# yilane/rag-project-icd10

Hardware: AMD Instinct MI355X
Metric: queries_per_sec (higher is better)
Workload: dtype f16; 1 GPU; BASELINE configs[1]: 10000 random fp32 768-d queries x 37000x768 corpus, top_k=10, search only (pre-embedded, HBM-resident inputs), level reweight fused; nq_per_gpu=10000, corpus_rows=37000, dim=768, top_k=10, mode=auto, parallelism=single GPU, collective_ranks=1

## Files before the change

### rag_project_icd10_amd/csrc/coarse_flat_kernel.hpp

```cpp
#pragma once
#include "coarse_common.hpp"
#include "flat_partition.hpp"

namespace icd {

struct CoarseFlatArgs {
    const _Float16 *q16;
    const _Float16 *c16;
    int nq;
    int n;
    int n_pad;
    int ctiles;
    int total_units;
    int units_per_wg;
    int pos_period;
    int list_tiles;
    int boot_tiles;
    int sparse_from;
    int P;
    float *part_scores;
    int *part_rows;
    float *bounds;
    unsigned int *shared_thr;
    const int *nq_ptr;
    const int *qlist;
    int nwg_virtual;
    int skip_below;
    unsigned long long *dbg;
    unsigned int *pace;
    int pace_period;
    int pace_epochs;
    int pace_shift;
    int pace_lead;
};

constexpr int CO_BOOT_MIN_TILES = 6;
constexpr int CO_KP_WIDE = 24;
constexpr int CO_BOOT_TILES = 8;
constexpr int PACE_SPIN_LIMIT = 20000;
constexpr int CO_SPARSE_FROM = 40;

template <int KP>
__device__ __forceinline__ float flush_emit_parallel(const char *smem, uint32_t qb, int h, int rot, int nlo, int nhi, float thr,
                                                      bool store, float *out_scores, int *out_rows) {
    constexpr int CAP = 64, HALF = 32;
    float v[HALF];
    uint32_t rw[HALF];
    const int lo_end = nlo, hi_begin = CAP - nhi;
#pragma unroll
    for (int j = 0; j < HALF; ++j) {
        const int slot = HALF * h + ((j + rot) & (HALF - 1));
        const bool valid = slot < lo_end || slot >= hi_begin;
        const float sv = *reinterpret_cast<const float *>(smem + qb + slot * 4);
        rw[j] = *reinterpret_cast<const uint32_t *>(smem + qb + CAP * 4 + slot * 4);
        v[j] = valid ? sv : -INFINITY;
    }
    auto pair_sum = [&](int x) {
        const auto sw = __builtin_amdgcn_permlane32_swap((unsigned)x, (unsigned)x, false, false);
        return x + (int)(h ? sw[0] : sw[1]);
    };
    const int total = nlo + nhi;
    float mx = -INFINITY;
#pragma unroll
    for (int j = 0; j < HALF; ++j) mx = fmaxf(mx, v[j]);
    {
        const auto sw = __builtin_amdgcn_permlane32_swap(__float_as_uint(mx), __float_as_uint(mx), false, false);
// ... 124 lines not shown
        quota_ties = h ? max(0, min(tied, room - min(tied_low_lane, room))) : min(tied, room);
        cut = tie;
    }
    int mine_n = 0;
#pragma unroll
    for (int j = 0; j < HALF; ++j) mine_n += (v[j] > cut) ? 1 : 0;
    mine_n += quota_ties;
    const auto swn = __builtin_amdgcn_permlane32_swap((unsigned)mine_n, (unsigned)mine_n, false, false);
    const int other_n = (int)(h ? swn[0] : swn[1]);
    if (total > KP) {
        int dest = h ? other_n : 0;
        int ties_left = quota_ties;
#pragma unroll
        for (int j = 0; j < HALF; ++j) {
            bool take = v[j] > cut;
            if (!take && ties_left > 0 && v[j] == tie && cnt_lo > KP) { take = true; --ties_left; }
            if (take) {
                *reinterpret_cast<float *>(smem + qb + dest * 4) = v[j];
                *reinterpret_cast<uint32_t *>(smem + qb + CAP * 4 + dest * 4) = rw[j];
                ++dest;
            }
        }
        const int kept = mine_n + other_n;
        st.thr = cut;
        st.kept = kept;
        st.aw0 = h ? qb + (CAP - 1) * 4 : qb + (uint32_t)kept * 4;
        st.aw = st.aw0;
    }
}

constexpr int CF_PRODUCT_VAR = 1 + 2 + 8 + 128 + 16 + 2048 + 32768;
constexpr int CF_CACHED_VAR = CF_PRODUCT_VAR + 2097152 + 4194304;
constexpr int CF_PACED_VAR = CF_PRODUCT_VAR + 67108864;
__host__ __device__ constexpr int cf_ring_stages(int var) { return (var & 1048576) ? 6 : CO_S; }
__host__ __device__ constexpr int cf_lds_bytes(int var) { return cf_ring_stages(var) * CO_STAGE_BYTES + CO_BM * CO_CAP * 8 + ((var & 1048576) ? 0 : 4 * 256); }
#define ICD_CF_STAMP(t) do { __builtin_amdgcn_sched_barrier(0); \
    asm volatile("s_memtime %0\n\ts_waitcnt lgkmcnt(0)" : "=s"(t) :: "memory"); \
    __builtin_amdgcn_sched_barrier(0); } while (0)

template <int D, int VAR = CF_PRODUCT_VAR, int KP = CO_KP, bool PERSIST = false>
__global__ __launch_bounds__(256, 1) void coarse_flat_kernel(CoarseFlatArgs a) {
    constexpr int CO_QUOTA = (CO_CAP - KP) / 2 - CO_CHECK_EVERY;
    static_assert(CO_QUOTA >= 8 && KP + 2 * (CO_QUOTA + CO_CHECK_EVERY) <= CO_CAP, "candidate buffer layout");
    constexpr bool EARLY_THR = (VAR & 1) != 0;
    constexpr bool DMA_SPREAD = (VAR & 2) != 0;
    constexpr bool Q_AGPR = (VAR & 8) != 0;
    constexpr bool PF2 = (VAR & 128) != 0;
    constexpr bool REV_WAIT = (VAR & 4) != 0;
    constexpr bool QUAD = (VAR & 16) != 0;
    constexpr bool SETPRIO = (VAR & 131072) != 0;
    constexpr int EXCH = (VAR & 524288) ? 4 : ((VAR & 262144) ? 2 : 1);
    constexpr bool X16 = (VAR & 32768) != 0;
    static_assert(!X16 || (QUAD && (VAR & 8) != 0 && D % 32 == 0), "the 16x16x32 form is built on the quad select and pinned queries");
    constexpr int EPOCH = ((VAR & 32) && (VAR & 2048)) ? 32 : ((VAR & 32) ? 16 : ((VAR & 2048) ? 24 : 0));
    constexpr bool NOBAR = (VAR & 256) != 0, NOVM = (VAR & 512) != 0, STAMPS = (VAR & 1024) != 0;
    constexpr bool NOPASS = (VAR & 4096) != 0, NOSEL = (VAR & 8192) != 0, NODMA = (VAR & 16384) != 0;
    constexpr bool PAIRBAR = (VAR & 1048576) != 0;
    constexpr bool DMA_WIDE = (VAR & 2097152) != 0;
    constexpr bool BOOT_MED3 = (VAR & 4194304) != 0;
    constexpr bool DIRTY_GUARD = (VAR & 8388608) != 0;
    constexpr bool SPARSE_PRE = (VAR & 16777216) != 0;
    static_assert(!SPARSE_PRE || (QUAD && X16), "the group pre-filter is built on the quad select of the 16x16x32 form");
    static_assert(!DMA_WIDE || (X16 && DMA_SPREAD && PF2 && !NODMA), "the wide spread is built on the product's 16x16x32 stage");
    constexpr bool CLOCKS = (VAR & 33554432) != 0;
    constexpr bool PACE = (VAR & 67108864) != 0;
    static_assert(!PACE || (EARLY_THR && EXCH == 1 && !PERSIST), "the pace poll rides on the early threshold load of every tile");
    static_assert(!(CLOCKS && STAMPS), "one use of the debug buffer at a time");
    constexpr int S = cf_ring_stages(VAR);
    constexpr int VM_MID = NOVM ? 63 : (PAIRBAR ? 4 : 4 * (S - 3));
    constexpr int PRO = PAIRBAR ? 4 : S - 1;
    constexpr int VM_TILE_END = NOVM ? 0 : (PAIRBAR ? (DMA_WIDE ? 6 : 8) : (DMA_WIDE ? 4 * (S - 2) - 2 : 4 * (S - 2)));
    constexpr int KS = D / CO_BK;
    constexpr int NF = D / 16;
    static_assert(KS % S == 0, "ring slot must be a compile-time function of the stage");
    using Ops = Sel2Ops<KP>;
    extern __shared__ __attribute__((aligned(16))) char smem[];

    const int tid = threadIdx.x, lane = tid & 63;
    const int wave = __builtin_amdgcn_readfirstlane(tid >> 6);
    const int c = lane & 31, h = lane >> 5;
    const int q16 = lane & 15, g16 = lane >> 4;
    const int nq_act = PERSIST && a.nq_ptr ? min(__builtin_amdgcn_readfirstlane(*a.nq_ptr), a.nq) : a.nq;
    const int total_units = PERSIST ? ((nq_act + CO_BM - 1) / CO_BM) * a.ctiles : a.total_units;
    const int nwg_logical = PERSIST ? (total_units + a.units_per_wg - 1) / a.units_per_wg : (int)gridDim.x;
    if (PERSIST && nq_act <= a.skip_below) return;
    unsigned long long clk_c0 = 0, clk_r0 = 0;
    if constexpr (CLOCKS) {
        clk_c0 = __builtin_amdgcn_s_memtime();
        clk_r0 = __builtin_amdgcn_s_memrealtime();
        __builtin_amdgcn_s_waitcnt(0xC07F);
    }

    uint32_t src_off[4];
#pragma unroll
    for (int i = 0; i < 4; ++i) {
        const int row_local = (wave * 4 + i) * 8 + (lane >> 3);
        const int piece = (lane & 7) ^ ((row_local >> 1) & 7);
        src_off[i] = (uint32_t)row_local * (uint32_t)(D * 2) + (uint32_t)piece * 16u - (uint32_t)(i * 1024);
    }
    uint32_t rd_off[4];
    if constexpr (X16) {
#pragma unroll
        for (int k2 = 0; k2 < 2; ++k2) rd_off[k2] = (uint32_t)q16 * 128u + (uint32_t)(((4 * k2 + g16) ^ ((q16 >> 1) & 7)) * 16);
        rd_off[2] = rd_off[3] = 0u;
    } else {
        const int sw = (c >> 1) & 7;
#pragma unroll
        for (int s = 0; s < 4; ++s) rd_off[s] = (uint32_t)c * 128u + (uint32_t)(((2 * s + h) ^ sw) * 16);
    }
    auto read_frags = [&](half8 (&f)[4], int ring_slot, int s) {
        if constexpr (X16) {
            const char *sb = smem + ring_slot * CO_STAGE_BYTES + (s & 1) * 8192 + rd_off[s >> 1];
#pragma unroll
            for (int t = 0; t < 4; ++t) f[t] = *reinterpret_cast<const half8 *>(sb + t * 2048);
        } else {
            const char *sb = smem + ring_slot * CO_STAGE_BYTES + rd_off[s];
#pragma unroll
            for (int t = 0; t < 4; ++t) f[t] = *reinterpret_cast<const half8 *>(sb + t * 4096);
        }
    };
    constexpr uint32_t RING_BYTES = (uint32_t)S * CO_STAGE_BYTES;
    const uint32_t wave_qbase = RING_BYTES + (uint32_t)(wave * 32) * Ops::QBYTES;
    const uint32_t wave_scratch = RING_BYTES + (uint32_t)CO_BM * Ops::QBYTES + (uint32_t)wave * 256u;
    unsigned long long st_vm = 0, st_bar = 0, st_body = 0, st_sel = 0, st_tiles = 0, st_prev = 0;
    unsigned long long st_comp[2] = {0, 0}, st_thr = 0, st_boot = 0;
    const int last_tile = a.ctiles - 1;

    half8 qf[NF];
    int cur_mtile = -1;
    for (int vblock = (int)blockIdx.x; vblock < (PERSIST ? nwg_logical : (int)blockIdx.x + 1); vblock += PERSIST ? (int)gridDim.x : 1) {
    const int wg = flat_workgroup_of_block(vblock, nwg_logical, a.pos_period);
    const int u_begin = wg * a.units_per_wg;
    const int u_end = min(total_units, u_begin + a.units_per_wg);
    if (u_begin >= u_end) continue;
    int u = u_begin;
    [[maybe_unused]] bool pacing = false;
    [[maybe_unused]] int pace_cls = 0, pace_members = 0, pace_last_epochs = 0;
    [[maybe_unused]] bool pace_last_mine = false;
    if constexpr (PACE) {
        if (a.pace && a.pace_period > 0) {
            pacing = true;
            pace_cls = wg % a.pace_period;
            pace_members = (nwg_logical - pace_cls + a.pace_period - 1) / a.pace_period;
            const int last_units = total_units - (nwg_logical - 1) * a.units_per_wg;
            pace_last_mine = ((nwg_logical - 1) % a.pace_period) == pace_cls;
            pace_last_epochs = last_units >> a.pace_shift;
        }
    }
    while (u < u_end) {
        const int mtile = u / a.ctiles;
        const int t0 = u - mtile * a.ctiles;
        const int run0 = max(u_begin - mtile * a.ctiles, 0);
        const int run1 = min(u_end - mtile * a.ctiles, a.ctiles);
        const int j = (t0 - run0) / a.list_tiles;
        const int t1 = min(run1, run0 + (j + 1) * a.list_tiles);
        const int ntiles = t1 - t0;
        const int ord = flat_first_ordinal(mtile, wg, a.ctiles, a.units_per_wg, a.list_tiles) + j;
        const int slot0 = mtile * CO_BM;

        if (mtile != cur_mtile) {
            if constexpr (X16) {
#pragma unroll
                for (int gr = 0; gr < 2; ++gr) {
                    int qr = slot0 + wave * 32 + 16 * gr + q16;
                    if (PERSIST && a.qlist) qr = a.qlist[min(qr, nq_act - 1)];
                    const _Float16 *qrow = a.q16 + (size_t)qr * D + 8 * g16;
#pragma unroll
                    for (int s = 0; s < NF / 2; ++s) qf[gr * (NF / 2) + s] = *reinterpret_cast<const half8 *>(qrow + 32 * s);
                }
            } else {
                int qr = slot0 + wave * 32 + c;
                if (PERSIST && a.qlist) qr = a.qlist[min(qr, nq_act - 1)];
                const _Float16 *qrow = a.q16 + (size_t)qr * D + 8 * h;
#pragma unroll
                for (int s = 0; s < NF; ++s) qf[s] = *reinterpret_cast<const half8 *>(qrow + 16 * s);
            }
            if constexpr (Q_AGPR) {
#pragma unroll
                for (int s = 0; s < NF; ++s) asm volatile("" : "+a"(qf[s]));
            }
            cur_mtile = mtile;
        }
        const __amdgpu_buffer_rsrc_t crsrc = __builtin_amdgcn_make_buffer_rsrc(
            const_cast<_Float16 *>(a.c16) + (size_t)t0 * CO_BN * D, 0,
            (int)min((size_t)(a.ctiles - t0) * CO_BN * (size_t)(D * 2), (size_t)0x7FFFFFFF), 0x00020000);
        auto issue_pieces = [&](int g_tile, int g_ks, int ring_slot, auto LO, auto HI) {
            const int trow = min(g_tile, last_tile - t0);
            char *dst = smem + ring_slot * CO_STAGE_BYTES + wave * 4096;
            const uint32_t soff = (uint32_t)trow * (uint32_t)(CO_BN * D * 2) + (uint32_t)g_ks * (CO_BK * 2);
            __attribute__((address_space(3))) void *ldst = (__attribute__((address_space(3))) void *)dst;
            constexpr int lo = decltype(LO)::value, hi = decltype(HI)::value;
            if constexpr (lo <= 0 && 0 < hi) __builtin_amdgcn_raw_ptr_buffer_load_lds(crsrc, ldst, 16, src_off[0], soff, 0, 0);
            if constexpr (lo <= 1 && 1 < hi) __builtin_amdgcn_raw_ptr_buffer_load_lds(crsrc, ldst, 16, src_off[1], soff, 1024, 0);
            if constexpr (lo <= 2 && 2 < hi) __builtin_amdgcn_raw_ptr_buffer_load_lds(crsrc, ldst, 16, src_off[2], soff, 2048, 0);
// ... 433 lines not shown
```

### rag_project_icd10_amd/csrc/finalize.hpp

```cpp
#pragma once
#include "exact_kernel.hpp"
#include "topk_select.hpp"

namespace icd {

constexpr int FIN_MAX_CAND = 512;
constexpr int FIN_MAX_CAND_X = 2048;
constexpr int FIN_MAX_K = 128;
constexpr int FIN_MAX_T = 256;
constexpr int FIN_EF = FIN_MAX_CAND / 64;
constexpr int FIN_EF_X = FIN_MAX_CAND_X / 64;
#ifndef ICD_FIN_WALK
#define ICD_FIN_WALK 8
#endif
constexpr int FIN_WALK = ICD_FIN_WALK;
#ifndef ICD_FIN_OCC
#define ICD_FIN_OCC 7
#endif

struct FinArgs {
    const float *part_scores;
    const int *part_rows;
    const float *bounds;
    long long perm_mul;
    int perm_mod;
    double perm_inv;
    int P, KP;
    int P_dense;
    int sparse_max;
    int dense_one_per_cu;
    int dense_grid, dense_bmq, dense_max_p, n_rows;
    int lds_cand;
    int lists_by_query;
    int skip_below;
    int narrow_check;
    int skip_walk;
    int wide_window;
    int nq;
    const int *nq_ptr;
    const int *qlist;
    int k;
    const float *queries;
    const float *corpus;
    int dim;
    const float *qnorm;
    const int *qexp;
    const unsigned char *qbad;
    float rmax, eps_rel;
    float rmax_unc, eps_f32;
    int cexp;
    int *nflag;
    int *flagged;
    float *thr0;
    int *counters;
    int track_run;
    int *host_counters;
    const int *levels;
    long long id_base;
    const long long *row_map;
    float *out_scores;
    long long *out_ids;
    double *out_adj;
    float *out_adj_raw;
    long long *out_adj_ids;
    int *out_adj_levels;
    const int *groups;
    int *out_levels;
    int *out_groups;
    int *out_adj_groups;
};

__device__ __forceinline__ double level_weight(int level) {
    return level == 1 ? 1.2 : (level == 3 ? 0.8 : 1.0);
}

__device__ __forceinline__ float wave_max_f32(float v) {
    const int ninf = (int)0xff800000u;
#define ICD_DPP_MAX(ctrl, rmask) v = fmaxf(v, __int_as_float(__builtin_amdgcn_update_dpp(ninf, __float_as_int(v), ctrl, rmask, 0xf, false)))
    ICD_DPP_MAX(0x111, 0xf);
    ICD_DPP_MAX(0x112, 0xf);
    ICD_DPP_MAX(0x114, 0xf);
    ICD_DPP_MAX(0x118, 0xf);
    ICD_DPP_MAX(0x142, 0xa);
    ICD_DPP_MAX(0x143, 0xc);
#undef ICD_DPP_MAX
// ... 268 lines not shown
        }
        return;
    }
    const int slot = blockIdx.x * 4 + wave;
    if (slot >= nq) return;
    const int qidx = a.qlist ? a.qlist[slot] : slot;
    if (qidx < 0) return;

    int P = a.P;
    if (a.nq_ptr && a.P_dense > 0 && nq > a.sparse_max)
        P = a.dense_max_p > 0 ? exact_adaptive_chunks(nq, a.dense_bmq, a.dense_grid, a.dense_max_p, a.n_rows, a.dense_one_per_cu) : a.P_dense;
    const int ncand = P * a.KP;
    const int lds_cand = a.lds_cand > 0 ? a.lds_cand : ncand;
    char *wbase = smem + (size_t)wave * fin_wave_lds_bytes(RESCORE, a.dim, lds_cand, EWM);
    u64 *keys = reinterpret_cast<u64 *>(wbase);
    u64 *sorted = keys + fin_key_slots(lds_cand);
    double *adjbuf = reinterpret_cast<double *>(sorted + fin_sorted_slots(EWM));
    float *qvec = reinterpret_cast<float *>(adjbuf + fin_adj_slots(EWM));
    float qn_early = 0.0f;
    int qexp_early = 0;
    unsigned char qbad_early = 0;
    if (RESCORE) {
        qn_early = a.qnorm[qidx];
        qexp_early = a.qexp[qidx];
        qbad_early = a.qbad[qidx];
        const float *qsrc0 = a.queries + (size_t)qidx * a.dim;
        for (int d = lane * 4; d < a.dim; d += 256)
            *reinterpret_cast<float4 *>(qvec + d) = *reinterpret_cast<const float4 *>(qsrc0 + d);
    }

    const int k = a.k;
    const size_t lslot = a.lists_by_query ? (size_t)qidx : (size_t)slot;
    const size_t pbase = lslot * ncand;

    const int T = !RESCORE ? k
                  : (a.wide_window && EWM >= 4) ? (ncand >= 256 ? 256 : (ncand >= 128 ? 128 : 64))
                  : ((EWM >= 4 && k > 64 && ncand >= 256) ? 256 : (EWM >= 2 && k > 32 && ncand >= 128) ? 128 : ((ncand > 128 && k <= 12) ? 32 : 64));
    float tau = -INFINITY;
    if (RESCORE) {
        if (lane < P) {
            const float bd = a.bounds[lslot * P + lane];
            if (bd > -INFINITY) tau = bd + fabsf(bd) * COARSE_KEY_SLACK;
        }
    }
    int nres = 0;
    bool merged = false;
    if constexpr (RESCORE && EWM >= 4) {
        if (T > 64) {
            const float two_eps = 2.0f * fin_eps(a, qn_early, qexp_early);
            nres = ncand <= 128 ? fin_merge_window<2>(a, pbase, ncand, T, k, two_eps, keys, sorted, lane, tau)
                                : fin_merge_window<FIN_EF>(a, pbase, ncand, T, k, two_eps, keys, sorted, lane, tau);
            merged = true;
        }
    }
    if (!merged) {
        int nvalid;
        if (ncand <= 128) nvalid = fin_merge<RESCORE, 2>(a, pbase, ncand, T, keys, sorted, lane, tau);
        else if (!RESCORE && EWM >= 4 && ncand > FIN_MAX_CAND) {
            if constexpr (!RESCORE && EWM >= 4) nvalid = fin_merge<false, FIN_EF_X>(a, pbase, ncand, T, keys, sorted, lane, tau);
            else nvalid = 0;
        }
        else nvalid = fin_merge<RESCORE, FIN_EF>(a, pbase, ncand, T, keys, sorted, lane, tau);
        nres = min(nvalid, T);
    }

    if (RESCORE) {
// ... 300 lines not shown
```

### rag_project_icd10_amd/csrc/icd_search.hip

```cpp
#include <hip/hip_runtime.h>

#include <algorithm>
#include <atomic>
#include <chrono>
#include <cmath>
#include <cstdarg>
#include <cstdio>
#include <cstring>
#include <mutex>
#include <new>
#include <string>
#include <vector>

#include "../../include/icd_search.h"
#include "coarse_flat_kernel.hpp"
#include "attention_kernel.hpp"
#include "exact_kernel.hpp"
#include "finalize.hpp"
#include "group_topk.hpp"
#include "hier_kernel.hpp"
#include "stats_kernel.hpp"
#include "stream_kernel.hpp"
#include "term_lookup.hpp"
#include "search_policy.hpp"
// ... 93 lines not shown
    int device = 0;
    bool opt_permute = true;
    bool opt_probe = true;
    bool opt_center = true;
    int opt_pace_shift = 3, opt_pace_lead = 2;
    bool opt_exact_narrow = true;
    int opt_host_one = 3;
    bool opt_stream_one = true;
    bool opt_family_order = true;
    int opt_wide_from = 48;
    int64_t n = 0, id_base = 0;
    long long *row_map = nullptr;
    int n_pad = 0;
    int dim = 0;
    int max_nq = 0, max_nq_pad = 0, max_k = 0;
    bool fast = false;
    float rmax = 0.f;
    float rmax_scaled = 0.f;
    int cexp = 0;
    float *cmean = nullptr;
    float rmax_unc_scaled = 0.f;
    float mean_share = 0.f;
    int num_cu = 256;
    float *corpus = nullptr;
    _Float16 *c16 = nullptr;
    int *levels = nullptr;
    float *qdev = nullptr;
    _Float16 *q16 = nullptr;
    float *qnorm = nullptr;
    int *qexp = nullptr;
    unsigned char *qbad = nullptr;
    float *thr0 = nullptr;
    unsigned int *shared_thr = nullptr;
    long long perm_mul = 0; int perm_mod = 0;
    float *partc_s = nullptr; int *partc_r = nullptr; float *partc_b = nullptr; size_t partc_cap = 0;
    float *part2_s = nullptr; int *part2_r = nullptr; float *part2_b = nullptr; size_t part2_cap = 0;
    float *partx_s = nullptr; int *partx_r = nullptr; size_t partx_cap = 0;
    float *lists_s = nullptr; int *lists_r = nullptr; size_t lists_cap = 0;
    int *nflag = nullptr; int *flagged = nullptr;
    int fallback_word = 0;
    int *h_nflag = nullptr;
    int *h_nflag_dev = nullptr;
    hipEvent_t ev_nflag = nullptr;
    unsigned int *scratch_u32 = nullptr;
    int *order = nullptr, *order_key = nullptr; unsigned int *order_hist = nullptr;
    float *o_scores = nullptr; long long *o_ids = nullptr;
    double *o_adj = nullptr; float *o_adj_raw = nullptr; long long *o_adj_ids = nullptr; int *o_adj_lv = nullptr;
    char *h_pin = nullptr, *h_pin_dev = nullptr;
    const float *host_q = nullptr;
    bool host_one_call = false;
    unsigned long long done_seq = 0;
    bool done_armed = false;
    size_t bytes_ws = 0;
    int chunks_override = 0;
    SearchPolicy pol;
    std::mutex mu;
    int probe_flagged = -1, probe_left = -1;
    bool pass2_enabled = true;
    bool adapt_enabled = true;
    bool profiling = false;
    int prof_every = 1;
    long prof_tick = 0;
    bool prof_now = false;
    bool capturing = false;
    hipEvent_t evring[EV_RING][NUM_EV + 1] = {};
    bool evring_valid[EV_RING][NUM_EV + 1] = {};
// ... 545 lines not shown
    x->fallback_word = 0;
    rec(x, 3, s);
    ExactArgs a{};
    a.corpus = x->corpus; a.queries = c.dq; a.nq = nq; a.n = (int)x->n; a.dim = x->dim; a.P = pn; a.strided = 1;
    a.rows_per_chunk = 128;
    a.part_scores = x->partx_s; a.part_rows = x->partx_r;
    int rc = launch_exact<32, 1, 4, 62, 16, 2, 16>(x, a, mtx_n, s);
    if (rc) return rc;
    rec(x, 4, s);
    FinArgs g = c.f;
    g.part_scores = x->partx_s; g.part_rows = x->partx_r; g.P = pn; g.KP = 32; g.nq = nq; g.lds_cand = pn * 32;
    g.narrow_check = 1; g.nflag = x->nflag; g.flagged = x->flagged;
    rc = launch_finalize<false>(x, g, s);
    if (rc) return rc;
    rec(x, 5, s);
    return run_exact(c, x->flagged, x->nflag, std::min(c.p_sparse, c.row_tiles), true, c.stream_ok, true, false, nullptr);
}

int search_exact(const SearchCtx &c) {
    icd_index *x = c.x;
    HIP_TRY(hipMemsetAsync(x->nflag, 0, sizeof(int), c.s));
    int px = pick_chunks(c.mtx, c.row_tiles, c.pmax_x, x->num_cu * c.wg_per_cu_x);
    const int rc = fit_chunks(c, &px);
    if (rc) return rc;
    x->last_chunks = px;
    rec(x, 3, c.s);
    return run_exact(c, nullptr, nullptr, px, true, false);
}

struct AutoPlan {
    bool wide_lists;
    bool wide_now;
    bool sparse_off;
    int kp_c;
    int ctiles, U, nwg;
    int pc;
    CoarseFlatArgs a;
    int p2, nwg2;
    CoarseFlatArgs a2;
};

int auto_prep(const SearchCtx &c, int nq_pad) {
    icd_index *x = c.x;
    ConvertArgs cv{};
    cv.src = c.dq; cv.dst = x->q16; cv.rows = c.nq; cv.rows_pad = nq_pad; cv.dim = x->dim; cv.mode = 0;
    cv.norm = x->qnorm; cv.scale_exp = x->qexp; cv.bad = x->qbad; cv.zero_u32 = x->shared_thr; cv.zero_i32 = x->nflag;
    cv.zero_u32b = x->shared_thr + x->max_nq_pad;
    hipLaunchKernelGGL(convert_rows_kernel, dim3((nq_pad + 3) / 4), dim3(256), 0, c.s, cv);
    HIP_TRY(hipGetLastError());
    rec(x, 1, c.s);
    return ICD_OK;
}

int split_class_period(int U, int ctiles, int nwg, int xcd_mode = -1) {
    int period = flat_class_period(U, ctiles);
    const int members = nwg / std::max(1, period);
    int split = (members + 11) / 12;
    if (xcd_mode == 0) period = 0;
    else if (xcd_mode == 1) period = 1 << 30;
    else if (xcd_mode == 2) split = 1;
    if (period > 0 && period < (1 << 20)) period *= std::max(1, split);
    return period;
}

int auto_plan(const SearchCtx &c, int nq_pad, AutoPlan &pl) {
    icd_index *x = c.x;
// ... 9 lines not shown
    const SearchDecision dec = policy_decide(x->pol, x->adapt_enabled, nq, k, x->chunks_override);
    pl.sparse_off = dec.sparse_off;
    pl.wide_now = dec.wide_now;
    pl.kp_c = pl.wide_lists ? CO_KP_WIDE : CO_KP;

    CoarseFlatArgs &a = pl.a;
    a = CoarseFlatArgs{};
    a.q16 = x->q16; a.c16 = x->c16; a.nq = nq; a.n = (int)x->n; a.n_pad = ctiles * 128; a.ctiles = ctiles;
    a.total_units = mtc * ctiles;
    a.boot_tiles = c.ov.flat_boot >= 0 ? c.ov.flat_boot : std::max(1, std::min(CO_BOOT_TILES, 96 / std::max(1, k)));
    a.sparse_from = c.ov.flat_sparse >= 0 ? c.ov.flat_sparse : CO_SPARSE_FROM;
    CoarsePlanIn pin{};
    pin.mtc = mtc; pin.ctiles = ctiles; pin.U = std::max(plan.U, c.ov.flat_u); pin.nq = nq; pin.k = k;
    pin.kp = pl.kp_c; pin.kp2 = CO_KP; pin.max_cand = FIN_MAX_CAND;
    pin.wide_lists = pl.wide_lists; pin.wide_now = pl.wide_now; pin.chunks_override = x->chunks_override;
    pin.pass2 = x->pass2_enabled && x->pol.pass2_armed() && x->part2_s;
    pin.partc_cap = (long long)x->partc_cap; pin.part2_cap = (long long)x->part2_cap;
    pin.max_list_tiles = flat_max_list_tiles(x->dim);
    if (c.ov.flat_list > 0) pin.list_override = c.ov.flat_list;
    const CoarsePlan cp = plan_coarse_lists(pin);
    if (!cp.ok)
        return fail(ICD_ERR_UNSUPPORTED, "coarse pass: no list plan for n=%lld dim=%d nq=%d k=%d (lists per query %d, at most %d tiles per list)",
                    (long long)x->n, x->dim, nq, k, cp.P, pin.max_list_tiles);
    const int U = cp.U;
    pl.U = U; pl.pc = cp.P;
    x->last_chunks = cp.P;
    pl.nwg = (a.total_units + U - 1) / U;
    a.list_tiles = cp.list_tiles;
    a.units_per_wg = U; a.P = cp.P;
    a.pos_period = split_class_period(U, ctiles, pl.nwg, c.ov.xcd_mode);
    a.part_scores = x->partc_s; a.part_rows = x->partc_r; a.bounds = x->partc_b; a.shared_thr = x->shared_thr;
    a.dbg = x->dbg;
    a.nwg_virtual = pl.nwg;
    pl.p2 = 0; pl.nwg2 = 0;
    pl.a2 = CoarseFlatArgs{};
    if (cp.P2 > 0) {
        const int U2 = cp.U2;
        CoarseFlatArgs &a2 = pl.a2;
        pl.p2 = cp.P2;
        a2 = a;
        a2.nq_ptr = nullptr; a2.qlist = nullptr;
        a2.units_per_wg = U2; a2.list_tiles = cp.list_tiles2; a2.P = pl.p2;
        a2.boot_tiles = a.boot_tiles;
        pl.nwg2 = (int)(((long long)mtc * ctiles + U2 - 1) / U2);
        a2.pos_period = split_class_period(U2, ctiles, pl.nwg2);
        a2.nwg_virtual = pl.nwg2;
        a2.part_scores = x->part2_s; a2.part_rows = x->part2_r; a2.bounds = x->part2_b;
        a2.shared_thr = x->shared_thr + x->max_nq_pad;
    }
    return ICD_OK;
}

int auto_coarse(const SearchCtx &c, AutoPlan &pl) {
    icd_index *x = c.x;
    hipStream_t s = c.s;
    CoarseFlatArgs &a = pl.a;
    const int nwg = pl.nwg;
    int rc;
    if (launch_coarse_variant(x, c.ov, a, nwg, s, &rc)) return rc;
    if (x->dim == 1024) return launch_coarse_flat<1024, (CF_PRODUCT_VAR & (3 | 16 | 2048))>(x, a, nwg, s);
    if (pl.wide_lists) return launch_coarse_flat<768, CF_PRODUCT_VAR, CO_KP_WIDE>(x, a, nwg, s);
    if ((size_t)x->n_pad * x->dim * 2 <= COARSE_CACHED_IMAGE_BYTES) return launch_coarse_flat<768, CF_CACHED_VAR>(x, a, nwg, s);
    const int t0 = flat_class_period(pl.U, pl.ctiles);
    const int members0 = t0 > 0 ? nwg / t0 : 0;
    const int epochs = x->opt_pace_shift >= 0 ? (pl.U >> x->opt_pace_shift) + 1 : 0;
    if (x->opt_pace_shift >= 0 && members0 >= 4 && (size_t)t0 * epochs <= PACE_WORDS) {
        a.pace = x->pace; a.pace_period = t0; a.pace_epochs = epochs; a.pace_shift = x->opt_pace_shift; a.pace_lead = std::max(1, x->opt_pace_lead);
        HIP_TRY(hipMemsetAsync(x->pace, 0, (size_t)t0 * epochs * sizeof(unsigned int), s));
    }
    return launch_coarse_flat<768, CF_PACED_VAR>(x, a, nwg, s);
}

int auto_first_finalize(const SearchCtx &c, const AutoPlan &pl, FinArgs &g, bool *wide_fin) {
    icd_index *x = c.x;
    const int nq = c.nq, k = c.k;
    hipStream_t s = c.s;
    g = c.f;
    g.part_scores = x->partc_s; g.part_rows = x->partc_r; g.bounds = x->partc_b; g.P = pl.pc; g.KP = pl.kp_c; g.nq = nq;
    g.perm_mul = x->perm_mul; g.perm_mod = x->perm_mod;
    g.perm_inv = (x->perm_mod > 0 && (double)x->perm_mod * (double)x->perm_mod < 9007199254740992.0) ? 1.0 / (double)x->perm_mod : 0.0;
    *wide_fin = pl.wide_now && k <= 32 && pl.pc * g.KP >= 128;
    if (*wide_fin) g.wide_window = 1;
    if (c.ov.fin_skip_walk) g.skip_walk = 1;
    if (*wide_fin && x->opt_family_order && nq >= 1024) {
        OrderArgs o{};
        o.part_scores = g.part_scores; o.part_rows = g.part_rows; o.P = g.P; o.KP = g.KP; o.nq = nq;
        o.perm_mul = g.perm_mul; o.perm_mod = g.perm_mod; o.perm_inv = g.perm_inv;
        o.shift = 6;
        while (((long long)x->n >> o.shift) >= ORDER_BUCKETS) ++o.shift;
        o.key = x->order_key; o.hist = x->order_hist; o.order = x->order;
        HIP_TRY(hipMemsetAsync(x->order_hist, 0, 2 * ORDER_BUCKETS * sizeof(unsigned int), s));
        hipLaunchKernelGGL(order_keys_kernel, dim3((nq + 3) / 4), dim3(256), 0, s, o);
        hipLaunchKernelGGL(order_scatter_kernel, dim3((nq + 1023) / 1024), dim3(1024), 0, s, o);
        HIP_TRY(hipGetLastError());
        g.qlist = x->order; g.lists_by_query = 1; g.nq = 4 * ((nq + 3) / 4);
    }
    const int rc = *wide_fin ? launch_finalize_t<true, false, 4>(x, g, s) : launch_finalize<true>(x, g, s);
    g.qlist = nullptr; g.lists_by_query = 0; g.nq = nq;
    return rc;
}

int auto_wide_retry(const SearchCtx &c, const FinArgs &g) {
    icd_index *x = c.x;
    FinArgs g2 = g;
    g2.qlist = x->flagged; g2.nq_ptr = x->nflag; g2.lists_by_query = 1; g2.wide_window = 1;
    g2.nflag = x->nflag + 1; g2.flagged = x->flagged + x->max_nq_pad;
    const int rc = launch_finalize_t<true, false, 4>(x, g2, c.s);
    if (rc) return rc;
    x->fallback_word = 1;
    return ICD_OK;
}

int auto_second_pass(const SearchCtx &c, AutoPlan &pl, const FinArgs &g) {
    icd_index *x = c.x;
    hipStream_t s = c.s;
    CoarseFlatArgs &a2 = pl.a2;
    const int w_in = x->fallback_word;
    a2.nq_ptr = x->nflag + w_in;
    a2.qlist = x->flagged + (size_t)w_in * x->max_nq_pad;
    a2.skip_below = PASS2_SKIP;
    const int grid2 = std::max(8, std::min(pl.nwg2, x->num_cu) & ~7);
    int rc;
    if (x->dim == 1024) rc = launch_coarse_flat<1024, (CF_PRODUCT_VAR & (3 | 16 | 2048)), CO_KP, true>(x, a2, grid2, s);
    else rc = launch_coarse_flat<768, CF_PRODUCT_VAR, CO_KP, true>(x, a2, grid2, s);
    if (rc) return rc;
    FinArgs g3 = g;
    g3.part_scores = x->part2_s; g3.part_rows = x->part2_r; g3.bounds = x->part2_b; g3.P = pl.p2; g3.KP = CO_KP;
    g3.qlist = a2.qlist; g3.nq_ptr = a2.nq_ptr; g3.lists_by_query = 0; g3.wide_window = 1; g3.skip_below = PASS2_SKIP;
    g3.nflag = x->nflag + 2; g3.flagged = x->flagged + (size_t)2 * x->max_nq_pad;
    rc = launch_finalize_t<true, false, 4>(x, g3, s);
    if (rc) return rc;
    x->fallback_word = 2;
    x->last_p2 = pl.p2; x->last_p2_word = w_in;
    return ICD_OK;
}

int auto_fallback(const SearchCtx &c, bool sparse_off) {
    icd_index *x = c.x;
    const int *fl_list = x->flagged + (size_t)x->fallback_word * x->max_nq_pad;
    const int *fl_count = x->nflag + x->fallback_word;
    int px = std::min(c.p_sparse, c.row_tiles);
    if (px < c.p_sparse) {
        const int rc = fit_chunks(c, &px);
        if (rc) return rc;
        return run_exact(c, fl_list, fl_count, px, true, false, true, true, c.f.thr0);
    }
    return run_exact(c, fl_list, fl_count, c.p_sparse, true, c.stream_ok, !sparse_off, true, c.f.thr0);
}

int search_auto(const SearchCtx &c) {
    icd_index *x = c.x;
    const int nq_pad = ((c.nq + 127) / 128) * 128;
    int rc = auto_prep(c, nq_pad);
    if (rc) return rc;
    AutoPlan pl;
    rc = auto_plan(c, nq_pad, pl);
    if (rc) return rc;
    rc = auto_coarse(c, pl);
    if (rc) return rc;
    rec(x, 2, c.s);
    FinArgs g;
    bool wide_fin = false;
    rc = auto_first_finalize(c, pl, g, &wide_fin);
    if (rc) return rc;
    x->fallback_word = 0;
    if (!wide_fin && c.k <= 32 && pl.pc * g.KP >= 128) {
        rc = auto_wide_retry(c, g);
        if (rc) return rc;
    }
    if (pl.p2 > 0) {
        rc = auto_second_pass(c, pl, g);
        if (rc) return rc;
    }
    policy_note_search(x->pol, x->adapt_enabled, x->pass2_enabled, c.nq, pl.p2, pl.wide_now, x->chunks_override, pl.pc * pl.kp_c);
    rec(x, 3, c.s);
    return auto_fallback(c, pl.sparse_off);
}

int search_device(icd_index *x, const float *dq, int nq, int k, int mode, const Outs &o, hipStream_t s, const BandArgs *band = nullptr, RowMasks mask = nullptr) {
    const bool use_fast = !band && (mode == ICD_MODE_AUTO) && x->fast && k <= FAST_MAX_K && (x->dim == 768 || x->dim == 1024);
    x->prof_now = !x->capturing && x->profiling && (x->prof_tick++ % x->prof_every == 0);
    if (x->prof_now) {
        const int slot = (int)(x->prof_count % EV_RING);
        x->ev = x->evring[slot];
        x->ev_valid = x->evring_valid[slot];
        ++x->prof_count;
        for (int i = 0; i <= NUM_EV; ++i) x->ev_valid[i] = false;
    }
    x->last_nq = nq;
    x->fallback_word = 0;
    x->last_p2 = 0;
    x->last_mode = use_fast ? ICD_MODE_AUTO : ICD_MODE_EXACT;
    rec(x, 0, s);
    const SearchCtx c = make_search_ctx(x, dq, nq, k, use_fast, o, s, band, mask);
    if (c.stream_ok && nq <= (use_fast ? (k <= 16 ? 16 : 0) : ST_MAX_ACTIVE)) return search_tiny(c);
    { const int rcq = stage_host_query(c); if (rcq) return rcq; }
    { const int rcb = stage_host_bands(c); if (rcb) return rcb; }
    if (!band && !use_fast && c.kpx > 32 && x->opt_exact_narrow && nq > ST_MAX_ACTIVE && c.row_tiles >= 64) {
        bool taken = false;
        const int rc = search_exact_narrow(c, &taken);
        if (rc || taken) return rc;
    }
    return use_fast ? search_auto(c) : search_exact(c);
}

// ... 111 lines not shown
        cv.rmax_bits = x->scratch_u32;
        if (x->cmean) cv.norm_raw_max = reinterpret_cast<float *>(x->scratch_u32 + 3);
        cv.perm_mul = x->perm_mul; cv.perm_mod = x->perm_mod;
        hipLaunchKernelGGL(convert_rows_kernel, dim3((x->n_pad + 3) / 4), dim3(256), 0, 0, cv);
        CR_TRY(hipGetLastError());
        CR_TRY(hipMemcpy(hv, x->scratch_u32, sizeof hv, hipMemcpyDeviceToHost));
        memcpy(&x->rmax_scaled, &hv[0], 4);
        x->rmax = ldexpf(x->rmax_scaled, -x->cexp);
        if (x->cmean) {
            float raw = 0.f;
            memcpy(&raw, &hv[3], 4);
            x->rmax = raw;
            x->rmax_unc_scaled = ldexpf(raw, x->cexp);
        }
        x->fast = (hv[1] == 0) && std::isfinite(x->rmax_scaled);
        if (!x->fast) { hipFree(x->c16); x->c16 = nullptr; }
    }
    if (x->fast) {
        CR_TRY(wsalloc(&x->q16, (size_t)x->max_nq_pad * dim));
        x->partc_cap = (size_t)coarse_partc_entries(x->max_nq_pad, std::min(max_k, FAST_MAX_K), CO_KP, CO_KP_WIDE, FIN_MAX_CAND);
        CR_TRY(wsalloc(&x->partc_s, x->partc_cap));
        CR_TRY(wsalloc(&x->partc_r, x->partc_cap));
        CR_TRY(wsalloc(&x->partc_b, x->partc_cap / CO_KP));
        x->part2_cap = (size_t)coarse_part2_entries(x->max_nq_pad, CO_KP);
        CR_TRY(wsalloc(&x->part2_s, x->part2_cap));
        CR_TRY(wsalloc(&x->part2_r, x->part2_cap));
        CR_TRY(wsalloc(&x->part2_b, x->part2_cap / CO_KP));
    }
    CR_TRY(wsalloc(&x->qnorm, (size_t)x->max_nq_pad));
    CR_TRY(wsalloc(&x->qexp, (size_t)x->max_nq_pad));
    CR_TRY(wsalloc(&x->qbad, (size_t)x->max_nq_pad));
    CR_TRY(wsalloc(&x->thr0, (size_t)x->max_nq_pad));
    CR_TRY(wsalloc(&x->shared_thr, (size_t)2 * x->max_nq_pad));
    CR_TRY(wsalloc(&x->qdev, (size_t)max_nq * dim));
    x->partx_cap = std::max<size_t>((size_t)x->max_nq_pad * 2 * exact_kp_for(max_k), (size_t)1 << 21);
    if (exact_kp_for(max_k) > 16)
        x->partx_cap = std::max<size_t>(x->partx_cap, (size_t)ST_MAX_ACTIVE * 512 * exact_kp_for(max_k));
    CR_TRY(wsalloc(&x->partx_s, x->partx_cap + (size_t)128 * FIN_MAX_CAND_X));
    CR_TRY(wsalloc(&x->partx_r, x->partx_cap + (size_t)128 * FIN_MAX_CAND_X));
    x->lists_cap = std::max((size_t)ST_MAX_ACTIVE * 1024 * exact_kp_for(max_k), (size_t)ST_FALLBACK_MAX_ACTIVE * 1024 * 16);
    CR_TRY(wsalloc(&x->lists_s, x->lists_cap));
    CR_TRY(wsalloc(&x->lists_r, x->lists_cap));
    CR_TRY(wsalloc(&x->nflag, 8));
    CR_TRY(hipMemset(x->nflag, 0, 8 * sizeof(int)));
    CR_TRY(hipHostMalloc(reinterpret_cast<void **>(&x->h_nflag), 8 * sizeof(int), hipHostMallocMapped));
    memset(x->h_nflag, 0, 8 * sizeof(int));
    CR_TRY(hipHostGetDevicePointer(reinterpret_cast<void **>(&x->h_nflag_dev), x->h_nflag, 0));
    CR_TRY(hipEventCreateWithFlags(&x->ev_nflag, hipEventDisableTiming));
    CR_TRY(hipHostMalloc(reinterpret_cast<void **>(&x->h_pin), PIN_Q_BYTES + PIN_OUT_BYTES + PIN_DONE_BYTES, hipHostMallocMapped));
    CR_TRY(hipHostGetDevicePointer(reinterpret_cast<void **>(&x->h_pin_dev), x->h_pin, 0));
    memset(x->h_pin + PIN_Q_BYTES + PIN_OUT_BYTES, 0, PIN_DONE_BYTES);
    CR_TRY(wsalloc(&x->band_dev, (size_t)max_nq));
    CR_TRY(hipHostMalloc(reinterpret_cast<void **>(&x->h_band), (size_t)max_nq * sizeof(BandQ), hipHostMallocDefault));
    if (!view_map) {
        CR_TRY(wsalloc(&x->mask_dev, (size_t)max_nq));
        CR_TRY(hipHostMalloc(reinterpret_cast<void **>(&x->h_mask), (size_t)max_nq * sizeof(uint32_t *), hipHostMallocDefault));
        CR_TRY(hipEventCreateWithFlags(&x->ev_mask, hipEventDisableTiming));
        const size_t mw = (size_t)rowmask_tile_words(n) + ROWMASK_TAIL_WORDS;
        std::vector<uint32_t> ones(mw, 0u);
        for (int64_t r = 0; r < n; r += 32) ones[(size_t)(r >> 5)] = n - r >= 32 ? ~0u : ((1u << (n - r)) - 1u);
        CR_TRY(wsalloc(&x->mask_ones, mw));
        CR_TRY(hipMemcpy(x->mask_ones, ones.data(), mw * sizeof(uint32_t), hipMemcpyHostToDevice));
    }
    CR_TRY(wsalloc(&x->pace, PACE_WORDS));
    CR_TRY(wsalloc(&x->dbg, (size_t)8192 * 16));
    CR_TRY(hipMemset(x->dbg, 0, (size_t)8192 * 16 * 8));
// ... 979 lines not shown
```

Baseline: 16.22 million queries/s.

## Fuse query fp32-to-fp16 prep into coarse kernel and clear thresholds in finalize

The separate query preparation pass (scale exponent, fp16 conversion, norm, bad flag) is folded into the coarse flat kernel's query-fragment load for dim 768. The kernel reads fp32 queries directly and converts them in registers. Owner blocks write q16, qnorm, qexp and qbad for the later stages. The shared-threshold buffer is now reset by the finalize kernels and tracked with a clean flag, which removes a memset, and the nflag zeroing moves into the kernel. This removes launches and a round trip through memory, but every column-tile block redoes the conversion work and the state handling becomes more complex.

```diff
diff --git a/rag_project_icd10_amd/csrc/coarse_flat_kernel.hpp b/rag_project_icd10_amd/csrc/coarse_flat_kernel.hpp
--- a/rag_project_icd10_amd/csrc/coarse_flat_kernel.hpp
+++ b/rag_project_icd10_amd/csrc/coarse_flat_kernel.hpp
@@ -32,6 +32,12 @@
     int pace_epochs;
     int pace_shift;
     int pace_lead;
+    const float *q32;
+    _Float16 *q16_out;
+    float *qnorm;
+    int *qexp;
+    unsigned char *qbad;
+    int *zero_i32;
 };
 
 constexpr int CO_BOOT_MIN_TILES = 6;
@@ -222,6 +228,7 @@
 constexpr int CF_PRODUCT_VAR = 1 + 2 + 8 + 128 + 16 + 2048 + 32768;
 constexpr int CF_CACHED_VAR = CF_PRODUCT_VAR + 2097152 + 4194304;
 constexpr int CF_PACED_VAR = CF_PRODUCT_VAR + 67108864;
+constexpr int CF_FUSED_PREP = 134217728;
 __host__ __device__ constexpr int cf_ring_stages(int var) { return (var & 1048576) ? 6 : CO_S; }
 __host__ __device__ constexpr int cf_lds_bytes(int var) { return cf_ring_stages(var) * CO_STAGE_BYTES + CO_BM * CO_CAP * 8 + ((var & 1048576) ? 0 : 4 * 256); }
 #define ICD_CF_STAMP(t) do { __builtin_amdgcn_sched_barrier(0); \
@@ -256,6 +263,8 @@
     constexpr bool PACE = (VAR & 67108864) != 0;
     static_assert(!PACE || (EARLY_THR && EXCH == 1 && !PERSIST), "the pace poll rides on the early threshold load of every tile");
     static_assert(!(CLOCKS && STAMPS), "one use of the debug buffer at a time");
+    constexpr bool FUSED_PREP = (VAR & 134217728) != 0;
+    static_assert(!FUSED_PREP || (X16 && !PERSIST), "the fused query prep is built on the first pass's 16x16x32 form");
     constexpr int S = cf_ring_stages(VAR);
     constexpr int VM_MID = NOVM ? 63 : (PAIRBAR ? 4 : 4 * (S - 3));
     constexpr int PRO = PAIRBAR ? 4 : S - 1;
@@ -316,6 +325,9 @@
     unsigned long long st_comp[2] = {0, 0}, st_thr = 0, st_boot = 0;
     const int last_tile = a.ctiles - 1;
 
+    if constexpr (FUSED_PREP) {
+        if (blockIdx.x == 0 && tid < 4) a.zero_i32[tid] = 0;
+    }
     half8 qf[NF];
     int cur_mtile = -1;
     for (int vblock = (int)blockIdx.x; vblock < (PERSIST ? nwg_logical : (int)blockIdx.x + 1); vblock += PERSIST ? (int)gridDim.x : 1) {
@@ -349,7 +361,65 @@
         const int slot0 = mtile * CO_BM;
 
         if (mtile != cur_mtile) {
-            if constexpr (X16) {
+            if constexpr (FUSED_PREP) {
+                const bool owner = run0 == 0;
+#pragma unroll
+                for (int gr = 0; gr < 2; ++gr) {
+                    const int qr = slot0 + wave * 32 + 16 * gr + q16;
+                    const bool real = qr < a.nq;
+                    const float *qrow = a.q32 + (size_t)(real ? qr : 0) * D + 8 * g16;
+                    float4 v[NF];
+#pragma unroll
+                    for (int s = 0; s < NF / 2; ++s) {
+                        v[2 * s] = *reinterpret_cast<const float4 *>(qrow + 32 * s);
+                        v[2 * s + 1] = *reinterpret_cast<const float4 *>(qrow + 32 * s + 4);
+                    }
+                    float m = 0.0f;
+                    bool bad = false;
+#pragma unroll
+                    for (int t = 0; t < NF; ++t) {
+                        if (!real) v[t] = float4{0.f, 0.f, 0.f, 0.f};
+                        const float f[4] = {v[t].x, v[t].y, v[t].z, v[t].w};
+#pragma unroll
+                        for (int i = 0; i < 4; ++i) {
+                            bad |= !(fabsf(f[i]) <= 3.402823466e38f);
+                            m = fmaxf(m, fabsf(f[i]));
+                        }
+                    }
+                    if (bad) m = INFINITY;
+                    m = fmaxf(m, __shfl_xor(m, 16));
+                    m = fmaxf(m, __shfl_xor(m, 32));
+                    const bool anybad = !(m <= 3.402823466e38f);
+                    const int e = anybad ? 0 : scale_exp_for(m);
+                    float ss = 0.0f;
+#pragma unroll
+                    for (int s = 0; s < NF / 2; ++s) {
+                        const float f[8] = {v[2 * s].x, v[2 * s].y, v[2 * s].z, v[2 * s].w, v[2 * s + 1].x, v[2 * s + 1].y, v[2 * s + 1].z, v[2 * s + 1].w};
+                        half8 hv;
+#pragma unroll
+                        for (int i = 0; i < 8; ++i) {
+                            const float x = ldexpf(f[i], e);
+                            ss = __builtin_fmaf(x, x, ss);
+                            hv[i] = (_Float16)x;
+                        }
+                        if (owner) *reinterpret_cast<half8 *>(a.q16_out + (size_t)qr * D + 8 * g16 + 32 * s) = hv;
+                        qf[gr * (NF / 2) + s] = hv;
+                        if constexpr (Q_AGPR) asm volatile("" : "+a"(qf[gr * (NF / 2) + s]));
+                    }
+                    if (owner) {
+                        ss += __shfl_xor(ss, 16);
+                        ss += __shfl_xor(ss, 32);
+                        if (real && g16 == 0) {
+                            float nrm = sqrtf(ss) * 1.000001f;
+                            if (!(nrm == nrm)) nrm = INFINITY;
+                            a.qnorm[qr] = nrm;
+                            a.qexp[qr] = e;
+                            a.qbad[qr] = anybad ? 1 : 0;
+                        }
+                    }
+                    __builtin_amdgcn_sched_barrier(0);
+                }
+            } else if constexpr (X16) {
 #pragma unroll
                 for (int gr = 0; gr < 2; ++gr) {
                     int qr = slot0 + wave * 32 + 16 * gr + q16;
diff --git a/rag_project_icd10_amd/csrc/finalize.hpp b/rag_project_icd10_amd/csrc/finalize.hpp
--- a/rag_project_icd10_amd/csrc/finalize.hpp
+++ b/rag_project_icd10_amd/csrc/finalize.hpp
@@ -51,6 +51,7 @@
     int cexp;
     int *nflag;
     int *flagged;
+    unsigned int *clear_thr;
     float *thr0;
     int *counters;
     int track_run;
@@ -385,6 +386,7 @@
     const int k = a.k;
     const size_t lslot = a.lists_by_query ? (size_t)qidx : (size_t)slot;
     const size_t pbase = lslot * ncand;
+    if (RESCORE && a.clear_thr && lane == 0) a.clear_thr[lslot] = 0u;
 
     const int T = !RESCORE ? k
                   : (a.wide_window && EWM >= 4) ? (ncand >= 256 ? 256 : (ncand >= 128 ? 128 : 64))
diff --git a/rag_project_icd10_amd/csrc/icd_search.hip b/rag_project_icd10_amd/csrc/icd_search.hip
--- a/rag_project_icd10_amd/csrc/icd_search.hip
+++ b/rag_project_icd10_amd/csrc/icd_search.hip
@@ -149,6 +149,7 @@
     unsigned char *qbad = nullptr;
     float *thr0 = nullptr;
     unsigned int *shared_thr = nullptr;
+    bool thr_clean = false;
     long long perm_mul = 0; int perm_mod = 0;
     float *partc_s = nullptr; int *partc_r = nullptr; float *partc_b = nullptr; size_t partc_cap = 0;
     float *part2_s = nullptr; int *part2_r = nullptr; float *part2_b = nullptr; size_t part2_cap = 0;
@@ -760,6 +761,7 @@
     bool wide_lists;
     bool wide_now;
     bool sparse_off;
+    bool fused_prep;
     int kp_c;
     int ctiles, U, nwg;
     int pc;
@@ -835,6 +837,9 @@
     a.part_scores = x->partc_s; a.part_rows = x->partc_r; a.bounds = x->partc_b; a.shared_thr = x->shared_thr;
     a.dbg = x->dbg;
     a.nwg_virtual = pl.nwg;
+    if (pl.fused_prep) {
+        a.q32 = c.dq; a.q16_out = x->q16; a.qnorm = x->qnorm; a.qexp = x->qexp; a.qbad = x->qbad; a.zero_i32 = x->nflag;
+    }
     pl.p2 = 0; pl.nwg2 = 0;
     pl.a2 = CoarseFlatArgs{};
     if (cp.P2 > 0) {
@@ -862,8 +867,8 @@
     int rc;
     if (launch_coarse_variant(x, c.ov, a, nwg, s, &rc)) return rc;
     if (x->dim == 1024) return launch_coarse_flat<1024, (CF_PRODUCT_VAR & (3 | 16 | 2048))>(x, a, nwg, s);
-    if (pl.wide_lists) return launch_coarse_flat<768, CF_PRODUCT_VAR, CO_KP_WIDE>(x, a, nwg, s);
-    if ((size_t)x->n_pad * x->dim * 2 <= COARSE_CACHED_IMAGE_BYTES) return launch_coarse_flat<768, CF_CACHED_VAR>(x, a, nwg, s);
+    if (pl.wide_lists) return launch_coarse_flat<768, CF_PRODUCT_VAR + CF_FUSED_PREP, CO_KP_WIDE>(x, a, nwg, s);
+    if ((size_t)x->n_pad * x->dim * 2 <= COARSE_CACHED_IMAGE_BYTES) return launch_coarse_flat<768, CF_CACHED_VAR + CF_FUSED_PREP>(x, a, nwg, s);
     const int t0 = flat_class_period(pl.U, pl.ctiles);
     const int members0 = t0 > 0 ? nwg / t0 : 0;
     const int epochs = x->opt_pace_shift >= 0 ? (pl.U >> x->opt_pace_shift) + 1 : 0;
@@ -871,7 +876,7 @@
         a.pace = x->pace; a.pace_period = t0; a.pace_epochs = epochs; a.pace_shift = x->opt_pace_shift; a.pace_lead = std::max(1, x->opt_pace_lead);
         HIP_TRY(hipMemsetAsync(x->pace, 0, (size_t)t0 * epochs * sizeof(unsigned int), s));
     }
-    return launch_coarse_flat<768, CF_PACED_VAR>(x, a, nwg, s);
+    return launch_coarse_flat<768, CF_PACED_VAR + CF_FUSED_PREP>(x, a, nwg, s);
 }
 
 int auto_first_finalize(const SearchCtx &c, const AutoPlan &pl, FinArgs &g, bool *wide_fin) {
@@ -898,8 +903,9 @@
         HIP_TRY(hipGetLastError());
         g.qlist = x->order; g.lists_by_query = 1; g.nq = 4 * ((nq + 3) / 4);
     }
+    if (pl.fused_prep) g.clear_thr = x->shared_thr;
     const int rc = *wide_fin ? launch_finalize_t<true, false, 4>(x, g, s) : launch_finalize<true>(x, g, s);
-    g.qlist = nullptr; g.lists_by_query = 0; g.nq = nq;
+    g.qlist = nullptr; g.lists_by_query = 0; g.nq = nq; g.clear_thr = nullptr;
     return rc;
 }
 
@@ -931,6 +937,7 @@
     g3.part_scores = x->part2_s; g3.part_rows = x->part2_r; g3.bounds = x->part2_b; g3.P = pl.p2; g3.KP = CO_KP;
     g3.qlist = a2.qlist; g3.nq_ptr = a2.nq_ptr; g3.lists_by_query = 0; g3.wide_window = 1; g3.skip_below = PASS2_SKIP;
     g3.nflag = x->nflag + 2; g3.flagged = x->flagged + (size_t)2 * x->max_nq_pad;
+    if (pl.fused_prep) g3.clear_thr = a2.shared_thr;
     rc = launch_finalize_t<true, false, 4>(x, g3, s);
     if (rc) return rc;
     x->fallback_word = 2;
@@ -954,11 +961,20 @@
 int search_auto(const SearchCtx &c) {
     icd_index *x = c.x;
     const int nq_pad = ((c.nq + 127) / 128) * 128;
-    int rc = auto_prep(c, nq_pad);
-    if (rc) return rc;
     AutoPlan pl;
+    pl.fused_prep = x->dim == 768 && !c.ov.has_flat_var;
+    int rc = ICD_OK;
+    const bool clean_after = x->thr_clean || !x->capturing;
+    if (pl.fused_prep) {
+        if (!x->thr_clean) HIP_TRY(hipMemsetAsync(x->shared_thr, 0, (size_t)2 * x->max_nq_pad * sizeof(unsigned int), c.s));
+        rec(x, 1, c.s);
+    } else {
+        rc = auto_prep(c, nq_pad);
+        if (rc) return rc;
+    }
     rc = auto_plan(c, nq_pad, pl);
     if (rc) return rc;
+    if (pl.fused_prep) x->thr_clean = false;
     rc = auto_coarse(c, pl);
     if (rc) return rc;
     rec(x, 2, c.s);
@@ -966,6 +982,7 @@
     bool wide_fin = false;
     rc = auto_first_finalize(c, pl, g, &wide_fin);
     if (rc) return rc;
+    if (pl.fused_prep && pl.p2 == 0) x->thr_clean = clean_after;
     x->fallback_word = 0;
     if (!wide_fin && c.k <= 32 && pl.pc * g.KP >= 128) {
         rc = auto_wide_retry(c, g);
@@ -974,6 +991,7 @@
     if (pl.p2 > 0) {
         rc = auto_second_pass(c, pl, g);
         if (rc) return rc;
+        if (pl.fused_prep) x->thr_clean = clean_after;
     }
     policy_note_search(x->pol, x->adapt_enabled, x->pass2_enabled, c.nq, pl.p2, pl.wide_now, x->chunks_override, pl.pc * pl.kp_c);
     rec(x, 3, c.s);
@@ -1151,6 +1169,8 @@
     CR_TRY(wsalloc(&x->qbad, (size_t)x->max_nq_pad));
     CR_TRY(wsalloc(&x->thr0, (size_t)x->max_nq_pad));
     CR_TRY(wsalloc(&x->shared_thr, (size_t)2 * x->max_nq_pad));
+    CR_TRY(hipMemset(x->shared_thr, 0, (size_t)2 * x->max_nq_pad * sizeof(unsigned int)));
+    x->thr_clean = true;
     CR_TRY(wsalloc(&x->qdev, (size_t)max_nq * dim));
     x->partx_cap = std::max<size_t>((size_t)x->max_nq_pad * 2 * exact_kp_for(max_k), (size_t)1 << 21);
     if (exact_kp_for(max_k) > 16)
```

New measurement: 15.82 million queries/s. -2.4%, worse.
